# EricLBuehler/mistral.rs

Hardware: AMD Instinct MI355X
Metric: decode_tokens_per_sec (higher is better)
Workload: dtype q4_k/q6_k weights x q8_k activations (int8 dot, f32 accumulate: the reference CPU path's arithmetic); 1 GPU; Llama-3-8B GGUF Q4_K_M, TP=1, 512 prefill / 1599 decode, batch 1, paged KV bf16 (block 32); parallelism=tp1

## Files before the change

mistral.rs_amd/csrc/dec_core2.cuh:

```cuda
#pragma once
#include "gguf_blocks.cuh"
#include <type_traits>
#include <utility>

#ifndef MRS_WAVE_SYNC
#define MRS_WAVE_SYNC() __builtin_amdgcn_wave_barrier()
#endif

namespace mrs {
namespace dec2 {

typedef unsigned v4u __attribute__((ext_vector_type(4)));
typedef unsigned v2u __attribute__((ext_vector_type(2)));
#ifndef MRS_DEC2_NT
#define MRS_DEC2_NT 512
#endif
constexpr int NT = MRS_DEC2_NT, NW = NT / 64;

__host__ __device__ inline bool dec_type(int t) { return t == T_Q4_K || t == T_Q5_K || t == T_Q6_K || t == T_Q8_0; }
enum : int { ACT_Q8K = 0, ACT_Q80 = 1 };
__host__ __device__ inline int act_mode_for(int type) { return type == T_Q8_0 ? ACT_Q80 : ACT_Q8K; }

struct Geo { int S, Cs, LPC, TPC, W, R, A; };
__host__ __device__ inline Geo geo_for(int K) {
  Geo g;
  g.S = K / 256;
  g.Cs = (g.S + 3) / 4;
  g.LPC = 4;
  g.TPC = g.Cs;
  g.W = 1;
  g.R = 4;
  g.A = 16;
  return g;
}
__host__ __device__ constexpr int slot_bytes(int type) { return type == T_Q4_K ? 148 : type == T_Q5_K ? 180 : type == T_Q6_K ? 210 : 272; }
__host__ __device__ constexpr unsigned tile_bytes(int type) { return 16u * (unsigned)slot_bytes(type); }
__host__ __device__ inline size_t rec_bytes(int type, const Geo &) { return tile_bytes(type); }
__host__ __device__ inline size_t tensor_bytes(int type, long long n, long long k) {
  const Geo g = geo_for((int)k);
  const size_t rgs = (size_t)((n + g.R - 1) / g.R);
  return rgs * g.TPC * (size_t)tile_bytes(type);
}

struct Mat {
  const uint8_t *base;
  unsigned bytes;
  int type, n, k;
};

template <int CTRL> __device__ __forceinline__ float dppf(float v) {
  return __builtin_bit_cast(float, __builtin_amdgcn_update_dpp(0, __builtin_bit_cast(int, v), CTRL, 0xf, 0xf, false));
}
template <int CTRL> __device__ __forceinline__ int dppi(int v) { return __builtin_amdgcn_update_dpp(0, v, CTRL, 0xf, 0xf, false); }
__device__ __forceinline__ float rlf(float v, int lane) { return __builtin_bit_cast(float, __builtin_amdgcn_readlane(__builtin_bit_cast(int, v), lane)); }
__device__ __forceinline__ float wave_max_all(float v) {
  v = fmaxf(v, dppf<0xB1>(v)); v = fmaxf(v, dppf<0x4E>(v)); v = fmaxf(v, dppf<0x141>(v)); v = fmaxf(v, dppf<0x140>(v));
  return fmaxf(fmaxf(rlf(v, 0), rlf(v, 16)), fmaxf(rlf(v, 32), rlf(v, 48)));
}
__device__ __forceinline__ int wave_min_all(int v) {
  v = min(v, dppi<0xB1>(v)); v = min(v, dppi<0x4E>(v)); v = min(v, dppi<0x141>(v)); v = min(v, dppi<0x140>(v));
  return min(min(__builtin_amdgcn_readlane(v, 0), __builtin_amdgcn_readlane(v, 16)), min(__builtin_amdgcn_readlane(v, 32), __builtin_amdgcn_readlane(v, 48)));
}
__device__ __forceinline__ float wave_sum_all(float v) {
  v += dppf<0xB1>(v); v += dppf<0x4E>(v); v += dppf<0x141>(v); v += dppf<0x140>(v);
  return (rlf(v, 0) + rlf(v, 16)) + (rlf(v, 32) + rlf(v, 48));
}
__device__ __forceinline__ float round_away(float x) { return truncf(x + copysignf(0.49999997f, x)); }
__device__ __forceinline__ float div_by(float x, float m, float y) {
  const float q0 = x * y;
  const float r = fmaf(-m, q0, x);
  return fmaf(r, y, q0);
}
__device__ __forceinline__ float4 as_f4(v4u v) { return make_float4(__uint_as_float(v.x), __uint_as_float(v.y), __uint_as_float(v.z), __uint_as_float(v.w)); }
__device__ __forceinline__ int dot16(v4u q, int4 u, int acc) { return dot4((int)q.w, u.w, dot4((int)q.z, u.z, dot4((int)q.y, u.y, dot4((int)q.x, u.x, acc)))); }
__device__ __forceinline__ int quad_sum(int v) { v += dppi<0xB1>(v); v += dppi<0x4E>(v); return v; }

constexpr int ACT_BS = 20;
__host__ __device__ inline int act_dw(int mode) { return mode == ACT_Q80 ? 12 : 1; }
__host__ __device__ inline int act_cq(int K) { return ((K / 256 + 3) / 4) * 256 + 16; }
__host__ __device__ inline int act_sp(int K) { return 4 * ((K / 256 + 3) / 4); }
__host__ __device__ inline size_t act_bytes(int K, int ncols) { return (size_t)ncols * ((size_t)4 * act_cq(K) + (size_t)act_sp(K) * (48 + ACT_BS * 4)); }
__host__ __device__ inline int chunk_of(int sb, int Cs) { return (sb >= Cs ? 1 : 0) + (sb >= 2 * Cs ? 1 : 0) + (sb >= 3 * Cs ? 1 : 0); }
struct Act {
  const char *q;
  const float *d;
  const int *bs;
  int K, S, dw, Cs, CQ, Sp;
  __device__ __forceinline__ int qoff(int sb) const { const int p = chunk_of(sb, Cs); return p * CQ + (sb - p * Cs) * 256; }
  __device__ __forceinline__ size_t qcol(int c) const { return (size_t)c * 4 * CQ; }
};
__device__ __forceinline__ Act act_view(char *smem, int K, int ncols, int mode) {
  const int S = K / 256, dw = act_dw(mode), CQ = act_cq(K), Sp = act_sp(K);
  char *d = smem + (size_t)ncols * 4 * CQ;
  return Act{smem, (const float *)d, (const int *)(d + (size_t)ncols * Sp * dw * 4), K, S, dw, (S + 3) / 4, CQ, Sp};
}

template <int N>
__device__ __forceinline__ void quantize_multi(const float4 (&v)[N], const int (&sb)[N], const bool (&live)[N], int c, int mode, char *img, int K, int ncols) {
  const int lane = lane_opaque(), S = K / 256, dw = act_dw(mode), Cs = (S + 3) / 4, CQ = act_cq(K), Sp = act_sp(K);
  char *q0p = img + (size_t)c * 4 * CQ;
  float *d0p = (float *)(img + (size_t)ncols * 4 * CQ) + (size_t)c * Sp * dw;
  int *b0p = (int *)(img + (size_t)ncols * 4 * CQ + (size_t)ncols * Sp * dw * 4) + (size_t)c * Sp * ACT_BS;
  int qo[N];
#pragma unroll
  for (int n = 0; n < N; ++n) { const int sbn = live[n] ? sb[n] : 0, p = chunk_of(sbn, Cs); qo[n] = p * CQ + (sbn - p * Cs) * 256; }
  if (mode == ACT_Q8K) {
    float amax[N], mx[N];
    bool tie = false;
#pragma unroll
    for (int n = 0; n < N; ++n) {
      const float hi4 = fmaxf(fmaxf(v[n].x, v[n].y), fmaxf(v[n].z, v[n].w)), lo4 = fminf(fminf(v[n].x, v[n].y), fminf(v[n].z, v[n].w));
      amax[n] = wave_max_all(fmaxf(hi4, -lo4));
      const unsigned long long bp = __ballot(hi4 == amax[n]), bn = __ballot(lo4 == -amax[n]);
      mx[n] = bn == 0 ? amax[n] : -amax[n];
      tie = tie || (bp != 0 && bn != 0 && amax[n] != 0.f);
    }
    if (tie) {
#pragma unroll
      for (int n = 0; n < N; ++n) {
        const int cand = fabsf(v[n].x) == amax[n] ? 0 : (fabsf(v[n].y) == amax[n] ? 1 : (fabsf(v[n].z) == amax[n] ? 2 : (fabsf(v[n].w) == amax[n] ? 3 : 1 << 20)));
        const int first = wave_min_all(lane * 4 + cand);
        const int sl = (first >> 2) & 63, comp = first & 3;
        const float m1 = rlf(comp == 0 ? v[n].x : (comp == 1 ? v[n].y : (comp == 2 ? v[n].z : v[n].w)), sl);
        mx[n] = amax[n] != 0.f ? m1 : mx[n];
      }
    }
#pragma unroll
    for (int n = 0; n < N; ++n) {
      const bool nz = amax[n] != 0.f;
      const float iscale = nz ? -128.f / mx[n] : 0.f;
      const int q0 = (int)fminf(127.f, round_away(iscale * v[n].x)), q1 = (int)fminf(127.f, round_away(iscale * v[n].y));
      const int q2 = (int)fminf(127.f, round_away(iscale * v[n].z)), q3 = (int)fminf(127.f, round_away(iscale * v[n].w));
      const float dd = nz ? 1.0f / iscale : 0.f;
      const int packed = (q0 & 0xff) | ((q1 & 0xff) << 8) | ((q2 & 0xff) << 16) | ((q3 & 0xff) << 24);
      int sum = dot4(packed, 0x01010101, 0);
      sum += dppi<0xB1>(sum);
      sum += dppi<0x4E>(sum);
      if (live[n]) {
        *(int *)(q0p + qo[n] + lane * 4) = packed;
        if ((lane & 3) == 0) b0p[(size_t)sb[n] * ACT_BS + (lane >> 2)] = sum;
        if (lane == 0) d0p[(size_t)sb[n] * dw] = dd;
      }
    }
  } else {
#pragma unroll
    for (int n = 0; n < N; ++n) {
      float amax = fmaxf(fmaxf(fabsf(v[n].x), fabsf(v[n].y)), fmaxf(fabsf(v[n].z), fabsf(v[n].w)));
      amax = fmaxf(amax, dppf<0xB1>(amax));
      amax = fmaxf(amax, dppf<0x4E>(amax));
      amax = fmaxf(amax, dppf<0x141>(amax));
      const float dq = amax / 127.0f, id = dq != 0.f ? 1.0f / dq : 0.0f;
      const int q0 = (int)round_away(v[n].x * id), q1 = (int)round_away(v[n].y * id), q2 = (int)round_away(v[n].z * id), q3 = (int)round_away(v[n].w * id);
      if (live[n]) {
        *(int *)(q0p + qo[n] + lane * 4) = (q0 & 0xff) | ((q1 & 0xff) << 8) | ((q2 & 0xff) << 16) | ((q3 & 0xff) << 24);
        if ((lane & 7) == 0) d0p[(size_t)sb[n] * dw + (lane >> 3)] = half_bits_to_float(float_to_half_bits(dq));
      }
    }
  }
}
__device__ __forceinline__ void quantize_sb(float4 v, int sb, int c, int mode, char *img, int K, int ncols) {
  const float4 va[1] = {v}; const int sa[1] = {sb}; const bool la[1] = {true};
  quantize_multi<1>(va, sa, la, c, mode, img, K, ncols);
}
__device__ __forceinline__ float4 norm4(float4 v, float4 w4, float nm, float inv) {
  v.x = div_by(v.x, nm, inv) * w4.x; v.y = div_by(v.y, nm, inv) * w4.y; v.z = div_by(v.z, nm, inv) * w4.z; v.w = div_by(v.w, nm, inv) * w4.w;
  return v;
}

constexpr int NPX = 7, NPW = 4;
template <int VW> struct ActRegs { v4u xv[VW][NPX]; v4u wv[VW][NPW]; };
template <int VW> __device__ __forceinline__ ActRegs<VW> act_issue_all(const void *x, unsigned xbytes, const float *nw, int K, int q) {
  ActRegs<VW> p;
  constexpr int P = 8 / VW;
  const int lane = lane_opaque();
  const __amdgpu_buffer_rsrc_t rx = __builtin_amdgcn_make_buffer_rsrc((void *)x, (short)0, (int)xbytes, 0x00020000);
  const __amdgpu_buffer_rsrc_t rw = __builtin_amdgcn_make_buffer_rsrc((void *)(nw ? (const void *)nw : x), (short)0, nw ? K * 4 : 0, 0x00020000);
  const int nv = (int)((xbytes + 8191u) / 8192u);
#pragma unroll
  for (int vw = 0; vw < VW; ++vw) {
    const unsigned off = (unsigned)((q + vw * P) * 64 + lane) * 16u;
#pragma unroll
    for (int j = 0; j < NPX; ++j) { p.xv[vw][j] = v4u{0u, 0u, 0u, 0u}; if (j < nv) p.xv[vw][j] = __builtin_amdgcn_raw_buffer_load_b128(rx, off + (unsigned)j * 8192u, 0, 0); }
  }
#pragma unroll
  for (int vw = 0; vw < VW; ++vw) {
    const unsigned off = (unsigned)((q + vw * P) * 64 + lane) * 16u;
#pragma unroll
    for (int j = 0; j < NPW; ++j) { p.wv[vw][j] = v4u{0u, 0u, 0u, 0u}; if (nw && j < nv) p.wv[vw][j] = __builtin_amdgcn_raw_buffer_load_b128(rw, off + (unsigned)j * 8192u, 0, 0); }
  }
  return p;
}
template <int NCOLS, int VW>
__device__ __forceinline__ void act_sumsq_all(float *red, const ActRegs<VW> &pre, const float *__restrict__ x, int ldx, const float *__restrict__ nw, int K, int q) {
  constexpr int P = 8 / VW;
  const int lane = lane_opaque();
  const int nv = (K + 2047) / 2048;
  if (!nw) return;
#pragma unroll
  for (int vw = 0; vw < VW; ++vw) {
    const int v = q + vw * P, vt = v * 64 + lane;
    auto ldx4 = [&](int c, int j) -> float4 { const int e = vt * 4 + j * 2048; return e < K ? *(const float4 *)(x + (size_t)c * ldx + e) : make_float4(0.f, 0.f, 0.f, 0.f); };
#pragma unroll
    for (int c = 0; c < NCOLS; ++c) {
      float ss = 0.f;
      auto sq = [&](float4 f) { ss = fmaf(f.x, f.x, ss); ss = fmaf(f.y, f.y, ss); ss = fmaf(f.z, f.z, ss); ss = fmaf(f.w, f.w, ss); };
#pragma unroll
      for (int j = 0; j < NPX; ++j) if (j < nv) sq(c == 0 ? as_f4(pre.xv[vw][j]) : ldx4(c, j));
      for (int j = NPX; j < nv; ++j) sq(ldx4(c, j));
      ss = wave_sum_all(ss);
      if (lane == 0) red[c * 8 + v] = ss;
    }
  }
}
template <int NCOLS, int VW>
__device__ __forceinline__ void act_quantize_all(char *img, const float *red, const ActRegs<VW> &pre, const float *__restrict__ x, int ldx, const float *__restrict__ nw, float eps, int K, int mode, int q,
                                                 int c0 = 0, int ncols_img = NCOLS) {
  constexpr int P = 8 / VW;
  const int lane = lane_opaque();
  const int nv = (K + 2047) / 2048;
#pragma unroll
  for (int c = 0; c < NCOLS; ++c) {
    float nm = 1.0f, inv = 1.0f;
    if (nw) {
      const float *r = red + c * 8;
      const float tot = ((r[0] + r[1]) + (r[2] + r[3])) + ((r[4] + r[5]) + (r[6] + r[7]));
      nm = sqrtf(tot / (float)K + eps);
      inv = 1.0f / nm;
    }
#pragma unroll
    for (int vw = 0; vw < VW; ++vw) {
      const int v = q + vw * P, vt = v * 64 + lane;
      auto ldx4 = [&](int j) -> float4 { const int e = vt * 4 + j * 2048; return e < K ? *(const float4 *)(x + (size_t)c * ldx + e) : make_float4(0.f, 0.f, 0.f, 0.f); };
      auto ldw4 = [&](int j) -> float4 { const int e = vt * 4 + j * 2048; return e < K ? *(const float4 *)(nw + e) : make_float4(0.f, 0.f, 0.f, 0.f); };
#pragma unroll
      for (int j0 = 0; j0 < NPX + 1; j0 += 4) {
        if (j0 < nv) {
          float4 vv[4]; int sb[4]; bool live[4];
#pragma unroll
          for (int i = 0; i < 4; ++i) {
            const int j = j0 + i;
            sb[i] = v + 8 * j; live[i] = j < nv && sb[i] * 256 < K;
            float4 xv = make_float4(0.f, 0.f, 0.f, 0.f), w4 = make_float4(0.f, 0.f, 0.f, 0.f);
            if (j < NPX) { xv = c == 0 ? as_f4(pre.xv[vw][j]) : (live[i] ? ldx4(j) : xv); } else if (live[i]) xv = ldx4(j);
            if (nw) { if (j < NPW) w4 = as_f4(pre.wv[vw][j]); else if (live[i]) w4 = ldw4(j); }
            vv[i] = nw ? norm4(xv, w4, nm, inv) : xv;
          }
          if (j0 + 2 < nv) quantize_multi<4>(vv, sb, live, c0 + c, mode, img, K, ncols_img);
          else {
            const float4 v2[2] = {vv[0], vv[1]}; const int s2[2] = {sb[0], sb[1]}; const bool l2[2] = {live[0], live[1]};
            quantize_multi<2>(v2, s2, l2, c0 + c, mode, img, K, ncols_img);
          }
        }
      }
      for (int j = NPX + 1; j < nv; ++j) {
        const int sb = v + 8 * j;
        if (sb * 256 < K) quantize_sb(nw ? norm4(ldx4(j), ldw4(j), nm, inv) : ldx4(j), sb, c0 + c, mode, img, K, ncols_img);
      }
    }
  }
}
template <int NCOLS>
__device__ __forceinline__ void act_finish_all(char *img, float *red, const ActRegs<1> &pre, const float *__restrict__ x, int ldx, const float *__restrict__ nw, float eps, int K, int mode, int q) {
  act_sumsq_all<NCOLS, 1>(red, pre, x, ldx, nw, K, q);
  if (nw) __syncthreads();
  act_quantize_all<NCOLS, 1>(img, red, pre, x, ldx, nw, eps, K, mode, q);
}
template <int VW> __device__ __forceinline__ void img_finish_all(char *smem, const ActRegs<VW> &pre, const void *img, size_t bytes, int q) {
  constexpr int P = 8 / VW;
  const int lane = lane_opaque();
#pragma unroll
  for (int vw = 0; vw < VW; ++vw) {
    const int vt = (q + vw * P) * 64 + lane;
#pragma unroll
    for (int j = 0; j < NPX; ++j) if ((size_t)(vt * 16 + j * 8192) < bytes) *(v4u *)(smem + vt * 16 + j * 8192) = pre.xv[vw][j];
    for (size_t o = (size_t)vt * 16 + (size_t)NPX * 8192; o < bytes; o += 8192) *(v4u *)(smem + o) = *(const v4u *)((const char *)img + o);
  }
}

#ifndef MRS_DEC2_LD_AUX
#define MRS_DEC2_LD_AUX 2
#endif
__device__ __forceinline__ v4u ldb128(__amdgpu_buffer_rsrc_t r, unsigned off) { return __builtin_amdgcn_raw_buffer_load_b128(r, off, 0, MRS_DEC2_LD_AUX); }
__device__ __forceinline__ v2u ldb64(__amdgpu_buffer_rsrc_t r, unsigned off) { return __builtin_amdgcn_raw_buffer_load_b64(r, off, 0, MRS_DEC2_LD_AUX); }
__device__ __forceinline__ unsigned ldb32(__amdgpu_buffer_rsrc_t r, unsigned off) { return __builtin_amdgcn_raw_buffer_load_b32(r, off, 0, MRS_DEC2_LD_AUX); }
__device__ __forceinline__ unsigned ldb16(__amdgpu_buffer_rsrc_t r, unsigned off) { return (unsigned)(unsigned short)__builtin_amdgcn_raw_buffer_load_b16(r, off, 0, MRS_DEC2_LD_AUX); }
__device__ __forceinline__ int byte_of(unsigned w, int i) { return (int)((w >> (8 * i)) & 0xffu); }
__device__ __forceinline__ int sbyte_of(unsigned w, int i) { return (int)(int8_t)((w >> (8 * i)) & 0xffu); }

#ifndef MRS_DEC2_NS_Q4K
#define MRS_DEC2_NS_Q4K 4
#endif
#ifndef MRS_DEC2_NS_Q5K
#define MRS_DEC2_NS_Q5K 4
#endif
#ifndef MRS_DEC2_NS_Q6K
#define MRS_DEC2_NS_Q6K 4
#endif
#ifndef MRS_DEC2_NS_Q80
#define MRS_DEC2_NS_Q80 4
#endif

struct ActQ { int4 a0, a1, a2, a3; };
__device__ __forceinline__ ActQ act_quarter(const Act &act, int col, int qo, int) {
  const char *qc = act.q + act.qcol(col) + qo;
  return ActQ{*(const int4 *)(qc), *(const int4 *)(qc + 16), *(const int4 *)(qc + 32), *(const int4 *)(qc + 48)};
}

template <int TYPE> struct Tile;

template <> struct Tile<T_Q4_K> {
  static constexpr int NS = MRS_DEC2_NS_Q4K;
  struct Raw { v4u q0, q1; unsigned hs, hd; };
  static __device__ __forceinline__ Raw load(__amdgpu_buffer_rsrc_t rs, unsigned tile, int lane) {
    Raw r;
    r.q0 = ldb128(rs, tile + (unsigned)lane * 16u);
    r.q1 = ldb128(rs, tile + 1024u + (unsigned)lane * 16u);
    r.hs = ldb32(rs, tile + 2048u + (unsigned)lane * 4u);
    r.hd = ldb32(rs, tile + 2304u + (unsigned)(lane >> 2) * 4u);
    return r;
  }
  template <int NCOLS> static __device__ __forceinline__ void term(const Raw &w, int sb, int qo, int c, const Act &act, int col0, float (&T)[NCOLS]) {
    const float d = half_bits_to_float((uint16_t)(w.hd & 0xffff)), dmin = half_bits_to_float((uint16_t)(w.hd >> 16));
    const v4u lo0 = w.q0 & 0x0F0F0F0Fu, hi0 = w.q0 & 0xF0F0F0F0u, lo1 = w.q1 & 0x0F0F0F0Fu, hi1 = w.q1 & 0xF0F0F0F0u;
    const int sca16 = byte_of(w.hs, 0) << 4, scb = byte_of(w.hs, 1), ma = byte_of(w.hs, 2), mb = byte_of(w.hs, 3);
#pragma unroll
    for (int k = 0; k < NCOLS; ++k) {
      const ActQ a = act_quarter(act, col0 + k, qo, c);
      const int4 b = *(const int4 *)(act.bs + ((size_t)(col0 + k) * act.Sp + sb) * ACT_BS + 4 * c);
      const int bsa = b.x + b.y, bsb = b.z + b.w;
      const int dlo = dot16(lo1, a.a1, dot16(lo0, a.a0, 0)), dhi = dot16(hi1, a.a3, dot16(hi0, a.a2, 0));
      const int isum16 = quad_sum(__mul24(sca16, dlo) + __mul24(scb, dhi + (bsb << 7)));
      const int msum = quad_sum(__mul24(ma, bsa) + __mul24(mb, bsb));
      const float yd = act.d[((size_t)(col0 + k) * act.Sp + sb) * act.dw];
      T[k] = fmaf(d * yd, (float)isum16 * 0.0625f, -((dmin * yd) * (float)msum));
    }
  }
};

template <> struct Tile<T_Q5_K> {
  static constexpr int NS = MRS_DEC2_NS_Q5K;
  struct Raw { v4u q0, q1; v2u xh; unsigned hs, hd; };
  static __device__ __forceinline__ Raw load(__amdgpu_buffer_rsrc_t rs, unsigned tile, int lane) {
    Raw r;
    r.q0 = ldb128(rs, tile + (unsigned)lane * 16u);
    r.q1 = ldb128(rs, tile + 1024u + (unsigned)lane * 16u);
    r.xh = ldb64(rs, tile + 2048u + (unsigned)lane * 8u);
    r.hs = ldb32(rs, tile + 2560u + (unsigned)lane * 4u);
    r.hd = ldb32(rs, tile + 2816u + (unsigned)(lane >> 2) * 4u);
    return r;
  }
  static __device__ __forceinline__ void fifth(v4u q, unsigned xh, v4u &lo, v4u &hi) {
    lo = q & 0x0F0F0F0Fu; hi = (q >> 4) & 0x0F0F0F0Fu;
    lo.x |= (xh & 0x01010101u) << 4; lo.y |= ((xh >> 1) & 0x01010101u) << 4; lo.z |= ((xh >> 2) & 0x01010101u) << 4; lo.w |= ((xh >> 3) & 0x01010101u) << 4;
    hi.x |= ((xh >> 4) & 0x01010101u) << 4; hi.y |= ((xh >> 5) & 0x01010101u) << 4; hi.z |= ((xh >> 6) & 0x01010101u) << 4; hi.w |= ((xh >> 7) & 0x01010101u) << 4;
  }
  template <int NCOLS> static __device__ __forceinline__ void term(const Raw &w, int sb, int qo, int c, const Act &act, int col0, float (&T)[NCOLS]) {
    const float d = half_bits_to_float((uint16_t)(w.hd & 0xffff)), dmin = half_bits_to_float((uint16_t)(w.hd >> 16));
    v4u lo0, hi0, lo1, hi1;
    fifth(w.q0, w.xh.x, lo0, hi0);
    fifth(w.q1, w.xh.y, lo1, hi1);
    const int sca = byte_of(w.hs, 0), scb = byte_of(w.hs, 1), ma = byte_of(w.hs, 2), mb = byte_of(w.hs, 3);
#pragma unroll
    for (int k = 0; k < NCOLS; ++k) {
      const ActQ a = act_quarter(act, col0 + k, qo, c);
      const int4 b = *(const int4 *)(act.bs + ((size_t)(col0 + k) * act.Sp + sb) * ACT_BS + 4 * c);
      const int bsa = b.x + b.y, bsb = b.z + b.w;
      const int dlo = dot16(lo1, a.a1, dot16(lo0, a.a0, 0)), dhi = dot16(hi1, a.a3, dot16(hi0, a.a2, 0));
      const int isum = quad_sum(__mul24(sca, dlo) + __mul24(scb, dhi));
      const int msum = quad_sum(__mul24(ma, bsa) + __mul24(mb, bsb));
      const float yd = act.d[((size_t)(col0 + k) * act.Sp + sb) * act.dw];
      T[k] = fmaf(d * yd, (float)isum, -((dmin * yd) * (float)msum));
    }
  }
};

template <> struct Tile<T_Q6_K> {
  static constexpr int NS = MRS_DEC2_NS_Q6K;
  struct Raw { v4u ql0, ql1, qh; unsigned sc, hd; };
  static __device__ __forceinline__ Raw load(__amdgpu_buffer_rsrc_t rs, unsigned tile, int lane) {
    Raw r;
    r.ql0 = ldb128(rs, tile + (unsigned)lane * 16u);
    r.ql1 = ldb128(rs, tile + 1024u + (unsigned)lane * 16u);
    r.qh = ldb128(rs, tile + 2048u + (unsigned)lane * 16u);
    r.sc = ldb32(rs, tile + 3072u + (unsigned)lane * 4u);
    r.hd = ldb16(rs, tile + 3328u + (unsigned)(lane >> 2) * 2u);
    return r;
  }
  template <int NCOLS> static __device__ __forceinline__ void term(const Raw &w, int sb, int qo, int c, const Act &act, int col0, float (&T)[NCOLS]) {
    const float d = half_bits_to_float((uint16_t)w.hd);
    const v4u h = w.qh;
    const v4u q0 = (w.ql0 & 0x0F0F0F0Fu) | ((h << 4) & 0x30303030u);
    const v4u q1 = ((w.ql0 >> 4) & 0x0F0F0F0Fu) | ((h << 2) & 0x30303030u);
    const v4u q2 = (w.ql1 & 0x0F0F0F0Fu) | (h & 0x30303030u);
    const v4u q3 = ((w.ql1 >> 4) & 0x0F0F0F0Fu) | ((h >> 2) & 0x30303030u);
    const int s0 = sbyte_of(w.sc, 0), s1 = sbyte_of(w.sc, 1), s2 = sbyte_of(w.sc, 2), s3 = sbyte_of(w.sc, 3);
#pragma unroll
    for (int k = 0; k < NCOLS; ++k) {
      const ActQ a = act_quarter(act, col0 + k, qo, c);
      const int4 b = *(const int4 *)(act.bs + ((size_t)(col0 + k) * act.Sp + sb) * ACT_BS + 4 * c);
      int iq = __mul24(s0, dot16(q0, a.a0, 0) - 32 * b.x) + __mul24(s1, dot16(q1, a.a1, 0) - 32 * b.y);
      iq += __mul24(s2, dot16(q2, a.a2, 0) - 32 * b.z) + __mul24(s3, dot16(q3, a.a3, 0) - 32 * b.w);
      const int isum = quad_sum(iq);
      const float yd = act.d[((size_t)(col0 + k) * act.Sp + sb) * act.dw];
      T[k] = (d * yd) * (float)isum;
    }
  }
};

template <> struct Tile<T_Q8_0> {
  static constexpr int NS = MRS_DEC2_NS_Q80;
  struct Raw { v4u q0, q1, q2, q3; unsigned dh; };
  static __device__ __forceinline__ Raw load(__amdgpu_buffer_rsrc_t rs, unsigned tile, int lane) {
    Raw r;
    r.q0 = ldb128(rs, tile + (unsigned)lane * 16u);
    r.q1 = ldb128(rs, tile + 1024u + (unsigned)lane * 16u);
    r.q2 = ldb128(rs, tile + 2048u + (unsigned)lane * 16u);
    r.q3 = ldb128(rs, tile + 3072u + (unsigned)lane * 16u);
    r.dh = ldb32(rs, tile + 4096u + (unsigned)lane * 4u);
    return r;
  }
  template <int NCOLS> static __device__ __forceinline__ void term(const Raw &w, int sb, int qo, int c, const Act &act, int col0, float (&T)[NCOLS]) {
    const float dwa = half_bits_to_float((uint16_t)(w.dh & 0xffff)), dwb = half_bits_to_float((uint16_t)(w.dh >> 16));
#pragma unroll
    for (int k = 0; k < NCOLS; ++k) {
      const ActQ a = act_quarter(act, col0 + k, qo, c);
      const float2 dx = *(const float2 *)(act.d + ((size_t)(col0 + k) * act.Sp + sb) * act.dw + 2 * c);
      const int isa = dot16(w.q1, a.a1, dot16(w.q0, a.a0, 0)), isb = dot16(w.q3, a.a3, dot16(w.q2, a.a2, 0));
      const float pa = (float)isa * dwa * dx.x, pb = (float)isb * dwb * dx.y;
      float r = pa + pb;
#pragma unroll
      for (int step = 1; step < 4; ++step) {
        const float prev = dppf<0x90>(r);
        const float cand = (prev + pa) + pb;
        r = c == step ? cand : r;
      }
      T[k] = dppf<0xFF>(r);
    }
  }
};

template <int TYPE, int NCOLS, int C0> struct TermCols {
  static __device__ __forceinline__ void run(const typename Tile<TYPE>::Raw &w, int sb, int qo, int c, const Act &act, int col0, float (&T)[NCOLS]) {
    if constexpr (C0 < NCOLS) {
      if constexpr (NCOLS - C0 >= 2) {
        float t2[2];
        Tile<TYPE>::template term<2>(w, sb, qo, c, act, col0 + C0, t2);
        T[C0] = t2[0]; T[C0 + 1] = t2[1];
      } else {
        float t1[1];
        Tile<TYPE>::template term<1>(w, sb, qo, c, act, col0 + C0, t1);
        T[C0] = t1[0];
      }
      if constexpr (C0 + 2 < NCOLS && (C0 & 2) != 0) __builtin_amdgcn_sched_barrier(0);
      TermCols<TYPE, NCOLS, C0 + 2>::run(w, sb, qo, c, act, col0, T);
    }
  }
};

struct Job {
  Mat mat[2];
  int nseg, rgpu;
  int nrows;
  int u0, u1;
  const int32_t *sel;
  int sel_mode;
  int upe;
  int ergs;
  unsigned long long *tl;
};
#define MRS_TL2(jb, i) do { if ((jb).tl && (tid_opaque() & 63) == 0) (jb).tl[((size_t)blockIdx.x * NW + (tid_opaque() >> 6)) * 16 + (i)] = __builtin_amdgcn_s_memrealtime(); } while (0)
__host__ __device__ inline int owner_off(const Geo &) { return 12; }
struct RecMeta { int ts_seg, row0, nvalid; };
struct NoAux {};

template <int TYPE, int NCOLS, bool SEGCOL = false, bool RING2 = false, class Stage, class AuxF, class Epi>
__device__ __forceinline__ void stream(const Job &jb, int K, int ncols_img, int mode, char *smem, int *ctr, bool sbar, Stage stage, AuxF auxf, Epi epi) {
  using TL = Tile<TYPE>;
  using AuxT = decltype(auxf(0));
  constexpr int NS = (NCOLS <= 4 && !RING2) ? TL::NS : (TL::NS > 2 ? 2 : TL::NS);
  const int tid = tid_opaque(), lane = tid & 63, wave = __builtin_amdgcn_readfirstlane(tid >> 6);
  const Geo g = geo_for(K);
  const int Cs = g.Cs;
  constexpr unsigned tileb = tile_bytes(TYPE);
  const int p = (lane >> 2) & 3, c = lane & 3;
  const int nun = jb.u1 - jb.u0 - wave;
  const int myunits = nun > 0 ? (nun + NW - 1) / NW : 0;
  const int tps = jb.rgpu * Cs;
  const int T = myunits * jb.nseg * tps;
  const int tpu = jb.nseg * tps;
  const bool dyn = tpu % NS == 0;
  if (tid == 0) *ctr = jb.u0 + NW;
  if (jb.u0 + wave >= jb.u1) {
    stage(0, wave);
    __syncthreads();
    stage(1, wave);
    if (sbar) __syncthreads();
    stage(2, wave);
    __syncthreads();
    return;
  }
  const __amdgpu_buffer_rsrc_t rs0 = __builtin_amdgcn_make_buffer_rsrc((void *)jb.mat[0].base, (short)0, (int)jb.mat[0].bytes, 0x00020000);
  const bool two = jb.nseg > 1;
  const __amdgpu_buffer_rsrc_t rs1 = __builtin_amdgcn_make_buffer_rsrc((void *)(two ? jb.mat[1].base : jb.mat[0].base), (short)0, (int)(two ? jb.mat[1].bytes : jb.mat[0].bytes), 0x00020000);
  typename TL::Raw ring[NS];
  RecMeta meta[NS];
  AuxT auxv[NS];
  unsigned long long selp = 0ull;
  const bool moe = jb.sel != nullptr;
  if (moe) {
    const int nsl = jb.sel_mode == 2 ? jb.nseg : min(8, (jb.u1 + jb.upe - 1) / jb.upe);
#pragma unroll
    for (int i = 0; i < 8; ++i) if (i < nsl) selp |= (unsigned long long)(unsigned)(__builtin_amdgcn_readfirstlane(jb.sel[i]) & 0xff) << (8 * i);
  }
  auto sel_at = [&](int i) { return (int)((selp >> (8 * (i & 7))) & 0xffull); };
  int lunit = 0, lseg = 0, lleft = 0, lts = 0, lrow0 = 0, lslot_row0 = 0;
  unsigned ltoff = 0, lubase1 = 0;
  auto open_unit = [&](int u) {
    lunit = u; lseg = 0; lts = 0; lleft = tps;
    if (u < jb.u1) {
      int local = u * jb.rgpu, e0 = 0, e1 = 0, sl = 0;
      if (moe) {
        if (jb.sel_mode == 2) { e0 = sel_at(0); e1 = sel_at(1); }
        else { sl = u / jb.upe; e0 = e1 = sel_at(sl); local -= sl * jb.upe * jb.rgpu; }
      }
      ltoff = (unsigned)(e0 * jb.ergs + local) * (unsigned)Cs * tileb;
      lubase1 = (unsigned)(e1 * jb.ergs + local) * (unsigned)Cs * tileb;
      lrow0 = u * jb.rgpu * g.R;
      lslot_row0 = sl * (jb.upe * jb.rgpu * g.R);
    }
  };
  constexpr unsigned DEAD = 0xF0000000u;
  auto issue = [&](typename TL::Raw &slot, RecMeta &m, AuxT &ax) {
    const bool livel = lunit < jb.u1;
    const int lrow = lrow0 - lslot_row0;
    m = RecMeta{livel ? (lts | (lseg << 24)) : -1, lrow0, min(g.R, jb.nrows - lrow)};
    slot = TL::load(lseg == 0 ? rs0 : rs1, livel ? ltoff : DEAD, lane);
    ax = auxf(livel ? lrow0 : 0);
    if (livel) {
      ltoff += tileb;
      if (++lts == Cs) { lts = 0; lrow0 += g.R; }
      if (--lleft == 0) {
        if (lseg + 1 < jb.nseg) { lseg = 1; lleft = tps; ltoff = lubase1; lrow0 -= jb.rgpu * g.R; }
        else if (dyn) {
          int nu = 0;
          if (lane == 0) nu = atomicAdd(ctr, 1);
          open_unit(__builtin_amdgcn_readfirstlane(nu));
        } else open_unit(lunit + NW);
      }
    }
  };
  open_unit(jb.u0 + wave);
  stage(0, wave);
  MRS_TL2(jb, 0);
  __syncthreads();
  issue(ring[0], meta[0], auxv[0]);
  stage(1, wave);
  if (sbar) __syncthreads();
  MRS_TL2(jb, 1);
#pragma unroll
  for (int i = 1; i < NS; ++i) issue(ring[i], meta[i], auxv[i]);
  stage(2, wave);
  MRS_TL2(jb, 2);
  __syncthreads();
  MRS_TL2(jb, 3);
  const Act act = act_view(smem, K, ncols_img, mode);
  const int pCs = p * Cs;
  const int qo_lane = p * act.CQ + c * 64;
  float acc[NCOLS];
#pragma unroll
  for (int k = 0; k < NCOLS; ++k) acc[k] = 0.0f;
  auto compute = [&](int i) {
    const int ts = meta[i].ts_seg & 0xffffff, seg = meta[i].ts_seg >> 24;
    const int sb = pCs + ts;
    const bool live = sb < g.S;
    float Tm[NCOLS];
    TermCols<TYPE, NCOLS, 0>::run(ring[i], sb, qo_lane + ts * 256, c, act, SEGCOL ? seg : 0, Tm);
#pragma unroll
    for (int k = 0; k < NCOLS; ++k) acc[k] = ts == 0 ? (live ? Tm[k] : 0.0f) : (live ? acc[k] + Tm[k] : acc[k]);
    if (ts == Cs - 1) {
      float tot[NCOLS];
#pragma unroll
      for (int k = 0; k < NCOLS; ++k) {
        float u = dppf<0x124>(acc[k]) + acc[k];
        u = dppf<0x124>(u) + acc[k];
        tot[k] = dppf<0x124>(u) + acc[k];
      }
      epi(seg, meta[i].row0, meta[i].nvalid, (meta[i].row0 / g.R) & (jb.rgpu - 1), tot, auxv[i]);
    }
  };
  if (dyn) {
    while (lunit < jb.u1) {
#pragma unroll
      for (int i = 0; i < NS; ++i) { compute(i); issue(ring[i], meta[i], auxv[i]); }
    }
#pragma unroll
    for (int i = 0; i < NS; ++i) compute(i);
  } else {
    const int rest = T > NS ? T - NS : 0;
    const int full = rest / NS;
    for (int ps = 0; ps < full; ++ps) {
#pragma unroll
      for (int i = 0; i < NS; ++i) { compute(i); issue(ring[i], meta[i], auxv[i]); }
    }
    if (rest - full * NS > 0) {
#pragma unroll
      for (int i = 0; i < NS; ++i) { compute(i); issue(ring[i], meta[i], auxv[i]); }
    }
#pragma unroll
    for (int i = 0; i < NS; ++i) if (meta[i].ts_seg >= 0) compute(i);
  }
  MRS_TL2(jb, 14);
}

}
}
```

mistral.rs_amd/csrc/dec_gemv.cuh:

```cuda
#pragma once
#include "dec_core2.cuh"
#include <algorithm>

namespace mrs {
namespace dec {
using namespace mrs::dec2;

enum : int { EPI_STORE = 0, EPI_RESID = 1, EPI_GLU = 2, EPI_QKV = 3, EPI_RESID2 = 4 };

struct GemvArgs {
  Mat m[3];
  int nrows[3];
  int K;
  const float *x; int ldx; const float *norm_w; float eps;
  float *out; int out_stride; float resid_scale;
  int activation;
  float *q_out; void *k_cache, *v_cache; const int64_t *slot_mapping; const int32_t *positions; const float *cos_t, *sin_t;
  int head_dim, rot_pairs, num_kv_heads, block_size, cache_x, kv_f16;
  int hd_shift, bs_shift, x_shift;
  int neox;
  int wg0[4];
  const int32_t *expert_sel;
  const float *acc_scale;
  int slots, slot_out_stride;
  const void *x_img;
  int units[3], rgpu;
  int ubase[3], urem[3], upe;
  unsigned long long *amax;
  unsigned long long *tl;
};
__device__ __forceinline__ unsigned long long pack_max_key(float v, int idx) {
  unsigned u = __float_as_uint(v);
  u = (u & 0x80000000u) ? ~u : (u | 0x80000000u);
  return ((unsigned long long)u << 32) | (unsigned)(0x7fffffff - idx);
}

enum : int { TM_Q4K = 1, TM_Q5K = 2, TM_Q6K = 4, TM_Q80 = 8, TM_ALL = 15 };
__host__ __device__ constexpr int tmask_of(int type) { return type == T_Q4_K ? TM_Q4K : type == T_Q5_K ? TM_Q5K : type == T_Q6_K ? TM_Q6K : type == T_Q8_0 ? TM_Q80 : 0; }
#define MRS_DEC_TYPE_SWITCH(t, ...)                                                              \
  switch (t) {                                                                                   \
  case T_Q4_K: if constexpr ((TMASK & TM_Q4K) != 0) { constexpr int TT = T_Q4_K; __VA_ARGS__ } break; \
  case T_Q5_K: if constexpr ((TMASK & TM_Q5K) != 0) { constexpr int TT = T_Q5_K; __VA_ARGS__ } break; \
  case T_Q6_K: if constexpr ((TMASK & TM_Q6K) != 0) { constexpr int TT = T_Q6_K; __VA_ARGS__ } break; \
  case T_Q8_0: if constexpr ((TMASK & TM_Q80) != 0) { constexpr int TT = T_Q8_0; __VA_ARGS__ } break; \
  default: break;                                                                                \
  }

template <int N> struct AuxV { float a[N], b[N]; };

template <int NCOLS, int EPI, int TMASK, bool RING2>
__device__ __forceinline__ void gemv_phase(const GemvArgs &a, char *smem, float *red, int *ctr, unsigned long long *best) {
  const int tid0 = tid_opaque();
  const int wave = __builtin_amdgcn_readfirstlane(tid0 >> 6), lane = tid0 & 63;
  const int K = a.K;
  const Geo g = geo_for(K);
  const int w1 = a.wg0[1], w2 = a.wg0[2], w3 = a.wg0[3];
  const int un0 = a.units[0], un1 = a.units[1], un2 = a.units[2];
  const int ub0 = a.ubase[0], ub1 = a.ubase[1], ub2 = a.ubase[2], ur0 = a.urem[0], ur1 = a.urem[1], ur2 = a.urem[2];
  const int nr0 = a.nrows[0], nr1 = a.nrows[1], nr2 = a.nrows[2];
  const uint8_t *b0 = a.m[0].base, *b1 = a.m[1].base, *b2 = a.m[2].base;
  const unsigned by0 = a.m[0].bytes, by1 = a.m[1].bytes, by2 = a.m[2].bytes;
  const int ty0 = a.m[0].type, ty1 = a.m[1].type, ty2 = a.m[2].type;
  const int bx = (int)blockIdx.x;
  int mi = 0;
  if constexpr (EPI == EPI_QKV) mi = bx >= w2 ? 2 : (bx >= w1 ? 1 : 0);
  const int wgb = EPI == EPI_QKV ? (mi == 0 ? 0 : (mi == 1 ? w1 : w2)) : 0;
  const int wge = EPI == EPI_QKV ? (mi == 0 ? w1 : (mi == 1 ? w2 : w3)) : (int)gridDim.x;
  const int units = EPI == EPI_QKV ? (mi == 0 ? un0 : (mi == 1 ? un1 : un2)) : un0;
  const int wi = bx - wgb;
  const int ub = EPI == EPI_QKV ? (mi == 0 ? ub0 : (mi == 1 ? ub1 : ub2)) : ub0, ur = EPI == EPI_QKV ? (mi == 0 ? ur0 : (mi == 1 ? ur1 : ur2)) : ur0;
  (void)wge; (void)units;
  Job jb{};
  jb.nseg = (EPI == EPI_GLU || EPI == EPI_RESID2) ? 2 : 1;
  jb.rgpu = a.rgpu;
  jb.mat[0].base = mi == 0 ? b0 : (mi == 1 ? b1 : b2);
  jb.mat[0].bytes = mi == 0 ? by0 : (mi == 1 ? by1 : by2);
  jb.mat[0].type = mi == 0 ? ty0 : (mi == 1 ? ty1 : ty2);
  jb.mat[0].n = 0; jb.mat[0].k = K;
  if constexpr (EPI == EPI_GLU) { jb.mat[1].base = b1; jb.mat[1].bytes = by1; jb.mat[1].type = ty1; jb.mat[1].n = 0; jb.mat[1].k = K; } else jb.mat[1] = jb.mat[0];
  jb.nrows = mi == 0 ? nr0 : (mi == 1 ? nr1 : nr2);
  jb.u0 = wi * ub + min(wi, ur); jb.u1 = jb.u0 + ub + (wi < ur ? 1 : 0);
  jb.sel = a.expert_sel; jb.sel_mode = EPI == EPI_RESID2 ? 2 : 1;
  jb.upe = a.upe;
  jb.ergs = (a.nrows[0] + g.R - 1) / g.R;
  jb.tl = a.tl;
  const int mode = act_mode_for(jb.mat[0].type);
  constexpr int NCI = EPI == EPI_RESID2 ? 2 : NCOLS;

  ActRegs<1> pre;
  const size_t img_bytes = act_bytes(K, NCI);
  const bool from_img = a.x_img != nullptr;
  const void *xsrc = from_img ? a.x_img : (const void *)a.x;
  const unsigned xbytes = from_img ? (unsigned)img_bytes : (unsigned)K * 4u;
  const float *nw_eff = from_img ? nullptr : a.norm_w;
  auto stage = [&](int st, int q) {
    if (st == 0) pre = act_issue_all<1>(xsrc, xbytes, nw_eff, K, q);
    else if (st == 1) act_sumsq_all<NCI, 1>(red, pre, a.x, a.ldx, nw_eff, K, q);
    else if (from_img) img_finish_all<1>(smem, pre, a.x_img, img_bytes, q);
    else act_quantize_all<NCI, 1>(smem, red, pre, a.x, a.ldx, a.norm_w, a.eps, K, mode, q);
  };
  const bool sbar = nw_eff != nullptr;
  constexpr bool AUX_RING = NCOLS == 1;
  const int lpr = 4 * g.LPC;
  const int rr = lane / lpr;
  const bool own = (lane & (lpr - 1)) == owner_off(g);
  if constexpr (EPI == EPI_STORE || EPI == EPI_RESID) {
    const float ascale = a.acc_scale ? *a.acc_scale : 1.0f;
    auto load_aux = [&](int row) {
      AuxV<NCOLS> v;
      const int rc = min(row, jb.nrows - 1);
#pragma unroll
      for (int c = 0; c < NCOLS; ++c) { v.a[c] = 0.f; v.b[c] = 0.f; if constexpr (EPI == EPI_RESID) v.a[c] = a.out[(size_t)c * a.out_stride + rc]; }
      return v;
    };
    auto auxf = [&](int row0) {
      if constexpr (AUX_RING) return load_aux(row0 + rr); else return NoAux{};
    };
    auto epi = [&](int, int row0, int nvalid, int, const float(&sum)[NCOLS], const auto &axr) {
      AuxV<NCOLS> ax;
      if constexpr (AUX_RING) ax = axr; else ax = load_aux(row0 + rr);
      if (own && rr < nvalid) {
#pragma unroll
        for (int c = 0; c < NCOLS; ++c) {
          float *o = a.out + (size_t)c * a.out_stride + row0 + rr;
          if constexpr (EPI == EPI_RESID) *o = ax.a[c] * a.resid_scale + sum[c] * ascale;
          else {
            *o = sum[c];
            if constexpr (NCOLS == 1) { if (a.amax) { const unsigned long long key = pack_max_key(sum[c], row0 + rr); *best = key > *best ? key : *best; } }
          }
        }
      }
    };
    MRS_DEC_TYPE_SWITCH(jb.mat[0].type, { stream<TT, NCOLS, false, RING2>(jb, K, NCI, mode, smem, ctr, sbar, stage, auxf, epi); })
  } else if constexpr (EPI == EPI_RESID2) {
    static_assert(EPI != EPI_RESID2 || NCOLS == 1, "one accumulator column; the image has two");
    const float w0 = a.acc_scale[0], w1 = a.acc_scale[1];
    float s0save = 0.0f;
    auto auxf = [&](int row0) {
      AuxV<1> v; v.a[0] = 0.f; v.b[0] = 0.f;
      const int row = row0 + rr;
      v.a[0] = a.out[min(row, jb.nrows - 1)];
      return v;
    };
    auto epi = [&](int seg, int row0, int nvalid, int, const float(&sum)[1], const AuxV<1> &ax) {
      if (seg == 0) {
        s0save = sum[0];
      } else if (own && rr < nvalid) {
        const float h1 = ax.a[0] * a.resid_scale + s0save * w0;
        a.out[row0 + rr] = h1 * 1.0f + sum[0] * w1;
      }
    };
    MRS_DEC_TYPE_SWITCH(jb.mat[0].type, { stream<TT, 1, true, RING2>(jb, K, NCI, mode, smem, ctr, sbar, stage, auxf, epi); })
  } else if constexpr (EPI == EPI_GLU) {
    float gsave[NCOLS];
#pragma unroll
    for (int c = 0; c < NCOLS; ++c) gsave[c] = 0.0f;
    auto auxf = [](int) { return NoAux{}; };
    auto epi = [&](int seg, int row0, int nvalid, int, const float(&sum)[NCOLS], const NoAux &) {
      if (seg == 0) {
#pragma unroll
        for (int c = 0; c < NCOLS; ++c) gsave[c] = sum[c];
      } else if (own && rr < nvalid) {
        const int row = row0 + rr;
        const int slot = a.slots > 1 ? row / a.nrows[0] : 0;
#pragma unroll
        for (int c = 0; c < NCOLS; ++c)
          a.out[(size_t)slot * a.slot_out_stride + (size_t)c * a.out_stride + (row - slot * a.nrows[0])] = (a.activation == 0 ? silu_engine(gsave[c]) : glu_act(gsave[c], a.activation)) * sum[c];
      }
    };
    MRS_DEC_TYPE_SWITCH(jb.mat[0].type, { stream<TT, NCOLS, false, RING2>(jb, K, NCI, mode, smem, ctr, sbar, stage, auxf, epi); })
  } else {
    int posv[NCOLS], slotv[NCOLS];
#pragma unroll
    for (int c = 0; c < NCOLS; ++c) { posv[c] = a.positions[c]; slotv[c] = mi == 0 ? 0 : (int)a.slot_mapping[c]; }
    auto load_aux = [&](int row) {
      AuxV<NCOLS> v;
      const int pair_i = (row & (a.head_dim - 1)) >> 1;
      const bool rot = mi < 2 && pair_i < a.rot_pairs;
      const int pi = min(pair_i, a.rot_pairs - 1);
#pragma unroll
      for (int c = 0; c < NCOLS; ++c) {
        const size_t ti = (size_t)posv[c] * a.rot_pairs + pi;
        const float cs = a.cos_t[ti], sn = a.sin_t[ti];
        v.a[c] = rot ? cs : 1.0f; v.b[c] = rot ? sn : 0.0f;
      }
      return v;
    };
    auto auxf = [&](int row0) {
      if constexpr (AUX_RING) return load_aux(row0 + rr); else return NoAux{};
    };
    float prev[NCOLS];
#pragma unroll
    for (int c = 0; c < NCOLS; ++c) prev[c] = 0.0f;
    auto epi = [&](int, int row0, int nvalid, int rgl, const float(&sum)[NCOLS], const auto &axr) {
      AuxV<NCOLS> ax;
      if constexpr (AUX_RING) ax = axr; else ax = load_aux(row0 + rr);
      const bool single = g.R == 1;
      if (single && (rgl & 1) == 0) {
#pragma unroll
        for (int c = 0; c < NCOLS; ++c) prev[c] = sum[c];
        return;
      }
      const int row = row0 + rr;
      const bool odd = single ? true : (row & 1) != 0;
      const int lr = single ? row - 1 : (row & ~1);
      const int head = lr >> a.hd_shift, dd = lr & (a.head_dim - 1);
      const bool nx = a.neox && mi < 2;
      const int d0 = nx ? dd >> 1 : dd, d1 = nx ? d0 + (a.head_dim >> 1) : dd + 1;
#pragma unroll
      for (int c = 0; c < NCOLS; ++c) {
        const float other = single ? prev[c] : __shfl(sum[c], lane ^ lpr, 64);
        const float xs = odd ? other : sum[c], ys = odd ? sum[c] : other;
        float x, y;
        rope_pair<float>(xs, ys, ax.a[c], ax.b[c], x, y);
        const bool wr0 = single ? own : (own && rr < nvalid && !odd), wr1 = single ? own : (own && rr < nvalid && odd);
        if (wr0 || wr1) {
          if (mi == 0) {
            if (wr0) a.q_out[(size_t)c * a.nrows[0] + head * a.head_dim + d0] = x;
            if (wr1) a.q_out[(size_t)c * a.nrows[0] + head * a.head_dim + d1] = y;
          } else {
            const int slot = slotv[c];
            if (slot >= 0) {
              const unsigned blk = (unsigned)slot >> a.bs_shift, off = (unsigned)slot & (unsigned)(a.block_size - 1);
              uint16_t *kc = (uint16_t *)a.k_cache, *vc = (uint16_t *)a.v_cache;
              const uint16_t xb = a.kv_f16 ? float_to_half_bits(x) : float_to_bf16_bits(x), yb = a.kv_f16 ? float_to_half_bits(y) : float_to_bf16_bits(y);
              if (mi == 1) {
                const int X = a.cache_x;
                const size_t hb = ((size_t)blk * a.num_kv_heads + head) * (size_t)(a.head_dim >> a.x_shift);
                if (wr0) kc[(hb + ((unsigned)d0 >> a.x_shift)) * a.block_size * X + off * X + ((unsigned)d0 & (unsigned)(X - 1))] = xb;
                if (wr1) kc[(hb + ((unsigned)d1 >> a.x_shift)) * a.block_size * X + off * X + ((unsigned)d1 & (unsigned)(X - 1))] = yb;
              } else {
                const size_t o = (((size_t)blk * a.num_kv_heads + head) * a.head_dim + dd) * a.block_size + off;
                if (wr0) vc[o] = xb;
                if (wr1) vc[o + a.block_size] = yb;
              }
            }
          }
        }
      }
    };
    MRS_DEC_TYPE_SWITCH(jb.mat[0].type, { stream<TT, NCOLS, false, RING2>(jb, K, NCI, mode, smem, ctr, sbar, stage, auxf, epi); })
  }
}

template <int NCOLS, int EPI, int TMASK = TM_ALL, bool RING2 = false>
__global__ void __launch_bounds__(NT) dec_gemv_kernel(const GemvArgs a) {
  extern __shared__ __attribute__((aligned(16))) char smem[];
  __shared__ float red[8 * 8];
  __shared__ int ctr;
  if constexpr (EPI == EPI_STORE && NCOLS == 1) {
    __shared__ unsigned long long wbest[NW];
    unsigned long long best = 0ull;
    gemv_phase<NCOLS, EPI, TMASK, RING2>(a, smem, red, &ctr, &best);
    if (a.amax) {
      const int tid = tid_opaque();
#pragma unroll
      for (int m = 32; m > 0; m >>= 1) { const unsigned long long o = __shfl_xor(best, m, 64); best = o > best ? o : best; }
      if ((tid & 63) == 0) wbest[tid >> 6] = best;
      __syncthreads();
      if (tid == 0) {
        unsigned long long b2 = wbest[0];
#pragma unroll
        for (int w = 1; w < NW; ++w) b2 = wbest[w] > b2 ? wbest[w] : b2;
        if (b2) atomicMax(a.amax, b2);
      }
    }
  } else gemv_phase<NCOLS, EPI, TMASK, RING2>(a, smem, red, &ctr, nullptr);
}


template <int NCOLS> int gemv_launch(int epi, int tmask, bool ring2, int grid, size_t lds, const GemvArgs &a, hipStream_t s);

}
}
```

Baseline: 532.8 tokens/s.

## Pipeline activation quantization in stages with weight tile compute in decode GEMV

For single-column store/residual GEMVs without a fused norm, the activation image in LDS is now quantized in chunks. Each chunk is published through a per-stage counter in LDS, so waves can start computing weight tiles on the first chunk while later chunks are still being built. This replaces the block-wide barrier that made every wave wait for the whole image, and the activation loads are remapped to a tiled sub-block layout so each stage covers contiguous sub-blocks. In exchange it adds spin-wait synchronisation in LDS and extra template variants, and correctness depends on the first passes only reading sub-blocks that are already built.

```diff
diff --git a/mistral.rs_amd/csrc/dec_core2.cuh b/mistral.rs_amd/csrc/dec_core2.cuh
--- a/mistral.rs_amd/csrc/dec_core2.cuh
+++ b/mistral.rs_amd/csrc/dec_core2.cuh
@@ -169,18 +169,28 @@
 
 constexpr int NPX = 7, NPW = 4;
 template <int VW> struct ActRegs { v4u xv[VW][NPX]; v4u wv[VW][NPW]; };
-template <int VW> __device__ __forceinline__ ActRegs<VW> act_issue_all(const void *x, unsigned xbytes, const float *nw, int K, int q) {
+__host__ __device__ inline int staged_sb(int v, int j, int S, int Cs) {
+  const int t = (v >> 2) + 2 * j, sb = (v & 3) * Cs + t;
+  return (t < Cs && sb < S) ? sb : -1;
+}
+template <int VW> __device__ __forceinline__ ActRegs<VW> act_issue_all(const void *x, unsigned xbytes, const float *nw, int K, int q, bool tiled = false) {
   ActRegs<VW> p;
   constexpr int P = 8 / VW;
   const int lane = lane_opaque();
   const __amdgpu_buffer_rsrc_t rx = __builtin_amdgcn_make_buffer_rsrc((void *)x, (short)0, (int)xbytes, 0x00020000);
   const __amdgpu_buffer_rsrc_t rw = __builtin_amdgcn_make_buffer_rsrc((void *)(nw ? (const void *)nw : x), (short)0, nw ? K * 4 : 0, 0x00020000);
   const int nv = (int)((xbytes + 8191u) / 8192u);
+  const int S = K / 256, Cs = (S + 3) / 4;
 #pragma unroll
   for (int vw = 0; vw < VW; ++vw) {
-    const unsigned off = (unsigned)((q + vw * P) * 64 + lane) * 16u;
-#pragma unroll
-    for (int j = 0; j < NPX; ++j) { p.xv[vw][j] = v4u{0u, 0u, 0u, 0u}; if (j < nv) p.xv[vw][j] = __builtin_amdgcn_raw_buffer_load_b128(rx, off + (unsigned)j * 8192u, 0, 0); }
+    const int v = q + vw * P;
+    const unsigned off = (unsigned)(v * 64 + lane) * 16u;
+#pragma unroll
+    for (int j = 0; j < NPX; ++j) {
+      p.xv[vw][j] = v4u{0u, 0u, 0u, 0u};
+      const int sbt = staged_sb(v, j, S, Cs);
+      if (tiled ? sbt >= 0 : j < nv) p.xv[vw][j] = __builtin_amdgcn_raw_buffer_load_b128(rx, tiled ? (unsigned)sbt * 1024u + (unsigned)lane * 16u : off + (unsigned)j * 8192u, 0, 0);
+    }
   }
 #pragma unroll
   for (int vw = 0; vw < VW; ++vw) {
@@ -265,6 +275,19 @@
   if (nw) __syncthreads();
   act_quantize_all<NCOLS, 1>(img, red, pre, x, ldx, nw, eps, K, mode, q);
 }
+constexpr int STAGE_TILES = 4, STAGES_MAX = (NPX + 1) / 2;
+__host__ __device__ inline int act_stages(int K) { return (((K / 256 + 3) / 4) + STAGE_TILES - 1) / STAGE_TILES; }
+__device__ __forceinline__ void act_quantize_stage(char *img, const ActRegs<1> &pre, int K, int mode, int q, int st) {
+  const int S = K / 256, Cs = (S + 3) / 4;
+  static_assert(NPX == 7, "four stages of two pieces, the last one holds one");
+  const v4u a = st == 0 ? pre.xv[0][0] : (st == 1 ? pre.xv[0][2] : (st == 2 ? pre.xv[0][4] : pre.xv[0][6]));
+  const v4u b = st == 0 ? pre.xv[0][1] : (st == 1 ? pre.xv[0][3] : (st == 2 ? pre.xv[0][5] : v4u{0u, 0u, 0u, 0u}));
+  const float4 v2[2] = {as_f4(a), as_f4(b)};
+  const int sa = staged_sb(q, 2 * st, S, Cs), sb = 2 * st + 1 < NPX ? staged_sb(q, 2 * st + 1, S, Cs) : -1;
+  const int s2[2] = {sa, sb};
+  const bool l2[2] = {sa >= 0, sb >= 0};
+  if (l2[0] || l2[1]) quantize_multi<2>(v2, s2, l2, 0, mode, img, K, 1);
+}
 template <int VW> __device__ __forceinline__ void img_finish_all(char *smem, const ActRegs<VW> &pre, const void *img, size_t bytes, int q) {
   constexpr int P = 8 / VW;
   const int lane = lane_opaque();
@@ -473,11 +496,29 @@
 struct RecMeta { int ts_seg, row0, nvalid; };
 struct NoAux {};
 
-template <int TYPE, int NCOLS, bool SEGCOL = false, bool RING2 = false, class Stage, class AuxF, class Epi>
-__device__ __forceinline__ void stream(const Job &jb, int K, int ncols_img, int mode, char *smem, int *ctr, bool sbar, Stage stage, AuxF auxf, Epi epi) {
+template <int TYPE, int NCOLS, bool SEGCOL = false, bool RING2 = false, bool STG = false, class Stage, class AuxF, class Epi>
+__device__ __forceinline__ void stream(const Job &jb, int K, int ncols_img, int mode, char *smem, int *ctr, bool sbar, bool staged_rt, Stage stage, AuxF auxf, Epi epi) {
   using TL = Tile<TYPE>;
   using AuxT = decltype(auxf(0));
   constexpr int NS = (NCOLS <= 4 && !RING2) ? TL::NS : (TL::NS > 2 ? 2 : TL::NS);
+  static_assert(!STG || (NCOLS == 1 && !SEGCOL && STAGE_TILES % NS == 0), "staged image build: one column, ring passes that divide a stage");
+  const bool staged = STG && staged_rt;
+  const int wave_u = __builtin_amdgcn_readfirstlane(tid_opaque() >> 6);
+  const int nst = act_stages(K);
+  auto build_stage = [&](int k) {
+    stage(3, wave_u, k);
+    __builtin_amdgcn_fence(__ATOMIC_RELEASE, "workgroup");
+    if (lane_opaque() == 0) atomicAdd(ctr + 1 + k, 1);
+  };
+  auto await_stage = [&](int k) {
+#if defined(__HIP_DEVICE_COMPILE__)
+    volatile __attribute__((address_space(3))) int *cp = (volatile __attribute__((address_space(3))) int *)(ctr + 1 + k);
+#else
+    volatile int *cp = ctr + 1 + k;
+#endif
+    while (__builtin_amdgcn_readfirstlane(*cp) < NW) __builtin_amdgcn_s_sleep(1);
+    __builtin_amdgcn_fence(__ATOMIC_ACQUIRE, "workgroup");
+  };
   const int tid = tid_opaque(), lane = tid & 63, wave = __builtin_amdgcn_readfirstlane(tid >> 6);
   const Geo g = geo_for(K);
   const int Cs = g.Cs;
@@ -490,12 +531,17 @@
   const int tpu = jb.nseg * tps;
   const bool dyn = tpu % NS == 0;
   if (tid == 0) *ctr = jb.u0 + NW;
+  if (STG && tid < STAGES_MAX) ctr[1 + tid] = 0;
   if (jb.u0 + wave >= jb.u1) {
-    stage(0, wave);
+    stage(0, wave, 0);
     __syncthreads();
-    stage(1, wave);
+    stage(1, wave, 0);
     if (sbar) __syncthreads();
-    stage(2, wave);
+    if (staged) {
+      for (int k = 0; k < nst; ++k) build_stage(k);
+      return;
+    }
+    stage(2, wave, 0);
     __syncthreads();
     return;
   }
@@ -550,19 +596,21 @@
     }
   };
   open_unit(jb.u0 + wave);
-  stage(0, wave);
+  stage(0, wave, 0);
   MRS_TL2(jb, 0);
   __syncthreads();
   issue(ring[0], meta[0], auxv[0]);
-  stage(1, wave);
+  stage(1, wave, 0);
   if (sbar) __syncthreads();
   MRS_TL2(jb, 1);
 #pragma unroll
   for (int i = 1; i < NS; ++i) issue(ring[i], meta[i], auxv[i]);
-  stage(2, wave);
-  MRS_TL2(jb, 2);
-  __syncthreads();
-  MRS_TL2(jb, 3);
+  if (!staged) {
+    stage(2, wave, 0);
+    MRS_TL2(jb, 2);
+    __syncthreads();
+    MRS_TL2(jb, 3);
+  }
   const Act act = act_view(smem, K, ncols_img, mode);
   const int pCs = p * Cs;
   const int qo_lane = p * act.CQ + c * 64;
@@ -588,6 +636,29 @@
       epi(seg, meta[i].row0, meta[i].nvalid, (meta[i].row0 / g.R) & (jb.rgpu - 1), tot, auxv[i]);
     }
   };
+  const int rest = T > NS ? T - NS : 0;
+  const int npass = (rest + NS - 1) / NS;
+  int ps = 0;
+  if (staged) {
+    for (int k = 0; k < nst; ++k) {
+      build_stage(k);
+      if (k + 1 == nst) MRS_TL2(jb, 2);
+      if (k + 1 < nst) {
+        await_stage(k);
+        if (k == 0) MRS_TL2(jb, 3);
+#pragma unroll
+        for (int r = 0; r < STAGE_TILES / NS; ++r) {
+          if (dyn ? lunit < jb.u1 : ps < npass) {
+            ++ps;
+#pragma unroll
+            for (int i = 0; i < NS; ++i) { compute(i); issue(ring[i], meta[i], auxv[i]); }
+          }
+        }
+      }
+    }
+    await_stage(nst - 1);
+    if (nst == 1) MRS_TL2(jb, 3);
+  }
   if (dyn) {
     while (lunit < jb.u1) {
 #pragma unroll
@@ -596,16 +667,10 @@
 #pragma unroll
     for (int i = 0; i < NS; ++i) compute(i);
   } else {
-    const int rest = T > NS ? T - NS : 0;
-    const int full = rest / NS;
-    for (int ps = 0; ps < full; ++ps) {
+    for (; ps < npass; ++ps) {
 #pragma unroll
       for (int i = 0; i < NS; ++i) { compute(i); issue(ring[i], meta[i], auxv[i]); }
     }
-    if (rest - full * NS > 0) {
-#pragma unroll
-      for (int i = 0; i < NS; ++i) { compute(i); issue(ring[i], meta[i], auxv[i]); }
-    }
 #pragma unroll
     for (int i = 0; i < NS; ++i) if (meta[i].ts_seg >= 0) compute(i);
   }
diff --git a/mistral.rs_amd/csrc/dec_gemv.cuh b/mistral.rs_amd/csrc/dec_gemv.cuh
--- a/mistral.rs_amd/csrc/dec_gemv.cuh
+++ b/mistral.rs_amd/csrc/dec_gemv.cuh
@@ -93,9 +93,12 @@
   const void *xsrc = from_img ? a.x_img : (const void *)a.x;
   const unsigned xbytes = from_img ? (unsigned)img_bytes : (unsigned)K * 4u;
   const float *nw_eff = from_img ? nullptr : a.norm_w;
-  auto stage = [&](int st, int q) {
-    if (st == 0) pre = act_issue_all<1>(xsrc, xbytes, nw_eff, K, q);
+  constexpr bool STG = NCOLS == 1 && (EPI == EPI_STORE || EPI == EPI_RESID) && (TMASK & TM_Q80) == 0;
+  const bool staged = STG && !from_img && a.norm_w == nullptr && g.Cs <= 2 * NPX;
+  auto stage = [&](int st, int q, int k) {
+    if (st == 0) pre = act_issue_all<1>(xsrc, xbytes, nw_eff, K, q, staged);
     else if (st == 1) act_sumsq_all<NCI, 1>(red, pre, a.x, a.ldx, nw_eff, K, q);
+    else if (st == 3) { if constexpr (STG) act_quantize_stage(smem, pre, K, mode, q, k); }
     else if (from_img) img_finish_all<1>(smem, pre, a.x_img, img_bytes, q);
     else act_quantize_all<NCI, 1>(smem, red, pre, a.x, a.ldx, a.norm_w, a.eps, K, mode, q);
   };
@@ -131,7 +134,7 @@
         }
       }
     };
-    MRS_DEC_TYPE_SWITCH(jb.mat[0].type, { stream<TT, NCOLS, false, RING2>(jb, K, NCI, mode, smem, ctr, sbar, stage, auxf, epi); })
+    MRS_DEC_TYPE_SWITCH(jb.mat[0].type, { stream<TT, NCOLS, false, RING2, STG>(jb, K, NCI, mode, smem, ctr, sbar, staged, stage, auxf, epi); })
   } else if constexpr (EPI == EPI_RESID2) {
     static_assert(EPI != EPI_RESID2 || NCOLS == 1, "one accumulator column; the image has two");
     const float w0 = a.acc_scale[0], w1 = a.acc_scale[1];
@@ -150,7 +153,7 @@
         a.out[row0 + rr] = h1 * 1.0f + sum[0] * w1;
       }
     };
-    MRS_DEC_TYPE_SWITCH(jb.mat[0].type, { stream<TT, 1, true, RING2>(jb, K, NCI, mode, smem, ctr, sbar, stage, auxf, epi); })
+    MRS_DEC_TYPE_SWITCH(jb.mat[0].type, { stream<TT, 1, true, RING2>(jb, K, NCI, mode, smem, ctr, sbar, false, stage, auxf, epi); })
   } else if constexpr (EPI == EPI_GLU) {
     float gsave[NCOLS];
 #pragma unroll
@@ -168,7 +171,7 @@
           a.out[(size_t)slot * a.slot_out_stride + (size_t)c * a.out_stride + (row - slot * a.nrows[0])] = (a.activation == 0 ? silu_engine(gsave[c]) : glu_act(gsave[c], a.activation)) * sum[c];
       }
     };
-    MRS_DEC_TYPE_SWITCH(jb.mat[0].type, { stream<TT, NCOLS, false, RING2>(jb, K, NCI, mode, smem, ctr, sbar, stage, auxf, epi); })
+    MRS_DEC_TYPE_SWITCH(jb.mat[0].type, { stream<TT, NCOLS, false, RING2>(jb, K, NCI, mode, smem, ctr, sbar, false, stage, auxf, epi); })
   } else {
     int posv[NCOLS], slotv[NCOLS];
 #pragma unroll
@@ -239,7 +242,7 @@
         }
       }
     };
-    MRS_DEC_TYPE_SWITCH(jb.mat[0].type, { stream<TT, NCOLS, false, RING2>(jb, K, NCI, mode, smem, ctr, sbar, stage, auxf, epi); })
+    MRS_DEC_TYPE_SWITCH(jb.mat[0].type, { stream<TT, NCOLS, false, RING2>(jb, K, NCI, mode, smem, ctr, sbar, false, stage, auxf, epi); })
   }
 }
 
@@ -247,11 +250,11 @@
 __global__ void __launch_bounds__(NT) dec_gemv_kernel(const GemvArgs a) {
   extern __shared__ __attribute__((aligned(16))) char smem[];
   __shared__ float red[8 * 8];
-  __shared__ int ctr;
+  __shared__ int ctr[1 + STAGES_MAX];
   if constexpr (EPI == EPI_STORE && NCOLS == 1) {
     __shared__ unsigned long long wbest[NW];
     unsigned long long best = 0ull;
-    gemv_phase<NCOLS, EPI, TMASK, RING2>(a, smem, red, &ctr, &best);
+    gemv_phase<NCOLS, EPI, TMASK, RING2>(a, smem, red, ctr, &best);
     if (a.amax) {
       const int tid = tid_opaque();
 #pragma unroll
@@ -265,7 +268,7 @@
         if (b2) atomicMax(a.amax, b2);
       }
     }
-  } else gemv_phase<NCOLS, EPI, TMASK, RING2>(a, smem, red, &ctr, nullptr);
+  } else gemv_phase<NCOLS, EPI, TMASK, RING2>(a, smem, red, ctr, nullptr);
 }
 
 
```

After: 517.2 tokens/s. -2.9%, worse.
